# femto-dev/femto

Measured on AMD Instinct MI355X. Metric: patterns/sec (count+locate) on 1 GiB index, higher is better.
Workload: dtype int64

## Files before the change

### femto_amd/build.py

```python
import os
import subprocess
from concurrent.futures import ThreadPoolExecutor

HERE = os.path.dirname(os.path.abspath(__file__))
CSRC = os.path.join(HERE, "csrc")
EXTRACT = os.path.join(HERE, "extract")
DOCLIST = os.path.join(HERE, "doclist")
DOCPOS = os.path.join(HERE, "docpos")
BQUERY = os.path.join(HERE, "bquery")
PLAN = os.path.join(HERE, "plan")
LINES = os.path.join(HERE, "lines")
SIMILAR = os.path.join(HERE, "similar")
MISMATCH = os.path.join(HERE, "mismatch")
EDIT = os.path.join(HERE, "edit")
CLASSES = os.path.join(HERE, "classes")
HAMMING = os.path.join(HERE, "hamming")
COMMON = os.path.join(HERE, "common")
OBJ = os.path.join(HERE, "_obj")
LIB = os.environ.get("FEMTO_AMD_LIB") or os.path.join(HERE, "libfemto_amd.so")
SOURCES = ["femto_amd_api.hip", "api_host.hip", "api_open.hip", "api_multi.hip", "regexp_search.hip", "resolve.hip", "trace_kernels.hip", "host_index.cpp", "index_builder.cpp", "suffix_sort.hip",
           "query_sort.hip", "host_pack.cpp", "../extract/extract.hip", "../doclist/doclist.hip", "../docpos/docpos.hip", "../bquery/bquery.hip", "../plan/plan_stream.hip", "../lines/lines.hip", "../similar/similar.hip", "../mismatch/mismatch.hip", "../edit/edit.hip", "../classes/classes.hip", "../hamming/hamming.hip"]
PLAIN_CXX = {"host_pack.cpp"}
CXX_FLAGS = ["-O3", "-std=c++17", "-fPIC", "-pthread"]
FLAGS = ["--offload-arch=gfx950", "-O3", "-std=c++17", "-fPIC", "-pthread", "-Wno-unused-result", "-Wno-cuda-compat"]
FLAGS += os.environ.get("FEMTO_AMD_EXTRA_FLAGS", "").split()
if os.environ.get("FEMTO_AMD_OBJ"):
    OBJ = os.environ["FEMTO_AMD_OBJ"]


def _headers():
    hs = [os.path.join(d, f) for d in (CSRC, EXTRACT, DOCLIST, DOCPOS, BQUERY, PLAN, LINES, SIMILAR, MISMATCH, EDIT, CLASSES, HAMMING, COMMON) for f in os.listdir(d) if f.endswith((".hpp", ".h"))]
    hs.append(os.path.join(os.path.dirname(HERE), "include", "femto_amd.h"))
    return hs


def _newest_header():
    return max(os.path.getmtime(h) for h in _headers())


def _obj(src):
    return os.path.join(OBJ, os.path.splitext(os.path.basename(src))[0] + ".o")


def _stale(src, hdr_time):
    o = _obj(src)
    if not os.path.exists(o):
        return True
    t = os.path.getmtime(o)
    return os.path.getmtime(os.path.join(CSRC, src)) > t or hdr_time > t


def needs_build():
    if not os.path.exists(LIB):
        return True
    t = os.path.getmtime(LIB)
    if _newest_header() > t:
        return True
    return any(os.path.getmtime(os.path.join(CSRC, f)) > t for f in SOURCES)


def build(force=False, verbose=False):
    if not force and not needs_build():
        return LIB
    os.makedirs(OBJ, exist_ok=True)
    hdr_time = _newest_header()
    todo = [s for s in SOURCES if force or _stale(s, hdr_time)]

    def compile_one(src):
        if src in PLAIN_CXX:
            cmd = ["hipcc"] + CXX_FLAGS + ["-x", "c++", "-c", os.path.join(CSRC, src), "-o", _obj(src)]
        else:
            cmd = ["hipcc"] + FLAGS + ["-x", "hip", "-c", os.path.join(CSRC, src), "-o", _obj(src)]
        if verbose:
            print(" ".join(cmd), flush=True)
        subprocess.run(cmd, check=True)

    with ThreadPoolExecutor(max_workers=min(8, max(1, len(todo)))) as ex:
        list(ex.map(compile_one, todo))
    cmd = ["hipcc", "--offload-arch=gfx950", "-fPIC", "-shared", "-pthread", "-o", LIB] + [_obj(s) for s in SOURCES]
    if verbose:
        print(" ".join(cmd), flush=True)
    subprocess.run(cmd, check=True)
    return LIB


TOOL_SRC = os.path.join(os.path.dirname(HERE), "tools", "femto_amd_multiquery.cpp")
TOOL = os.path.join(HERE, "femto_amd_multiquery")


SEARCH_SRC = os.path.join(os.path.dirname(HERE), "tools", "femto_amd_search.cpp")
SEARCH = os.path.join(HERE, "femto_amd_search")


def build_tools(force=False, verbose=False):
    for src, exe in ((TOOL_SRC, TOOL), (SEARCH_SRC, SEARCH)):
        if not force and os.path.exists(exe) and os.path.getmtime(exe) > max(os.path.getmtime(src), os.path.getmtime(LIB)):
            continue
        cmd = ["g++", "-std=c++17", "-O2", "-o", exe, src, "-L" + HERE, "-lfemto_amd", "-Wl,-rpath,$ORIGIN",
               "-Wl,-rpath-link," + HERE, "-Wl,--allow-shlib-undefined"]
        if verbose:
            print(" ".join(cmd))
        subprocess.run(cmd, check=True)
    return TOOL


if __name__ == "__main__":
    build(force=True, verbose=True)
    build_tools(force=True, verbose=True)
```

### femto_amd/plan/plan_stream.hip

```cpp
#include <algorithm>
#include <atomic>
#include <cstdlib>

#include "../csrc/api_internal.hpp"
#include "../csrc/kernels.hip.hpp"
#include "../csrc/pack_kernels.hip.hpp"
#include "../csrc/ru_kernels.hip.hpp"
#include "../csrc/pack2_kernels.hip.hpp"
#include "../csrc/ind_kernels.hip.hpp"
#include "../csrc/text_kernels.hip.hpp"
#include "../csrc/ctx_kernels.hip.hpp"
#include "../csrc/direct_kernels.hip.hpp"
#include "plan_span.hpp"

namespace femto_amd {
namespace {

struct alignas(16) I64x2 { int64_t x, y; };

__device__ __forceinline__ void wave_lds_sync() {
  __builtin_amdgcn_fence(__ATOMIC_RELEASE, "wavefront");
  __builtin_amdgcn_wave_barrier();
  __builtin_amdgcn_fence(__ATOMIC_ACQUIRE, "wavefront");
}

__device__ __forceinline__ int4 load_counts(const int32_t* __restrict__ noccs, int64_t npats, int64_t t, int64_t t1, int lane) {
  int4 v = make_int4(0, 0, 0, 0);
  if (t >= t1) return v;
  const int64_t q0 = t * kPlanTile + 4 * lane;
  if (q0 + 4 <= npats) {
    v = *reinterpret_cast<const int4*>(noccs + q0);
  } else {
    if (q0 < npats) v.x = noccs[q0];
    if (q0 + 1 < npats) v.y = noccs[q0 + 1];
    if (q0 + 2 < npats) v.z = noccs[q0 + 2];
  }
  return v;
}

__device__ __forceinline__ void load_quad(const int64_t* __restrict__ a, bool vec, int64_t q0, const bool need[4], int64_t out[4]) {
  if (vec) {
    const I64x2 lo = *reinterpret_cast<const I64x2*>(a + q0), hi = *reinterpret_cast<const I64x2*>(a + q0 + 2);
    out[0] = lo.x; out[1] = lo.y; out[2] = hi.x; out[3] = hi.y;
  } else {
#pragma unroll
    for (int j = 0; j < 4; j++) out[j] = need[j] ? a[q0 + j] : 0;
  }
}

template <bool kLong>
__global__ __launch_bounds__(256) __attribute__((amdgpu_waves_per_eu(kLong ? 6 : 8, 8))) void plan_stream_kernel(
    const int64_t npats, const int32_t* __restrict__ noccs, const int64_t* __restrict__ first, const PlanSums ps,
    int64_t* __restrict__ out_starts, int64_t* __restrict__ offsets, const int64_t capacity, int* __restrict__ big_flag,
    const DevIndex ix, int64_t* __restrict__ total_out, int64_t* __restrict__ total_user, const int64_t* __restrict__ sa_known) {
  __shared__ uint32_t s_incl[kPlanWavesPerGroup][kPlanTile];
  __shared__ int64_t s_first[kPlanWavesPerGroup][kPlanTile];
  __shared__ int64_t s_lrel[kLong ? kPlanWavesPerGroup : 1][kLong ? kPlanTile : 1];
  const int lane = threadIdx.x & 63, wv = threadIdx.x >> 6;
  const int64_t nwaves = int64_t(gridDim.x) * kPlanWavesPerGroup, wave = int64_t(blockIdx.x) * kPlanWavesPerGroup + wv;
  for (int64_t k = wave * 64 + lane; k < ps.next_words; k += nwaves * 64) ps.next_super[k] = 0;
  const PlanSpan span = plan_span_of(ps.nblocks, nwaves, wave);
  if (span.t0 >= span.t1) return;
  int4 cur = load_counts(noccs, npats, span.t0, span.t1, lane);
  int4 nx1 = load_counts(noccs, npats, span.t0 + 1, span.t1, lane);
  int64_t base;
  {
    const int64_t b = span.t0, g = b >> 6;
    uint64_t acc = lane < int(b & 63) ? uint64_t(ps.sums[(b & ~int64_t(63)) + lane]) : 0;
    if (lane < int(g & 63)) acc += uint64_t(ps.super[(g & ~int64_t(63)) + lane]);
    for (int64_t k = lane; k < (g >> 6); k += 64) acc += uint64_t(ps.super2[k]);
    const uint64_t part = wave_sum_u64(acc);
    const uint32_t lo = uint32_t(__shfl(int(uint32_t(part)), 0, 64)), hi = uint32_t(__shfl(int(uint32_t(part >> 32)), 0, 64));
    base = int64_t((uint64_t(hi) << 32) | lo);
  }
  const bool first_vec = (reinterpret_cast<uintptr_t>(first) & 15u) == 0, known_vec = (reinterpret_cast<uintptr_t>(sa_known) & 15u) == 0;
  for (int64_t t = span.t0; t < span.t1; t++) {
    const int4 nx2 = load_counts(noccs, npats, t + 2, span.t1, lane);
    const int64_t q0 = t * kPlanTile + 4 * lane;
    const int64_t n[4] = {int64_t(cur.x), int64_t(cur.y), int64_t(cur.z), int64_t(cur.w)};
    const int64_t lsum = n[0] + n[1] + n[2] + n[3];
    int64_t incl = lsum;
    if (kLong) {
      uint64_t v = uint64_t(lsum);
#pragma unroll
      for (int d = 1; d < 64; d <<= 1) {
        const uint32_t lo = uint32_t(__shfl_up(int(uint32_t(v)), d, 64)), hi = uint32_t(__shfl_up(int(uint32_t(v >> 32)), d, 64));
        if (lane >= d) v += (uint64_t(hi) << 32) | lo;
      }
      incl = int64_t(v);
    } else {
      uint32_t v = uint32_t(lsum);
#pragma unroll
      for (int d = 1; d < 64; d <<= 1) {
        const uint32_t y = uint32_t(__shfl_up(int(v), d, 64));
        if (lane >= d) v += y;
      }
      incl = int64_t(v);
    }
    int64_t tile_rows;
    if (kLong) {
      const uint32_t lo = uint32_t(__shfl(int(uint32_t(uint64_t(incl))), 63, 64)), hi = uint32_t(__shfl(int(uint32_t(uint64_t(incl) >> 32)), 63, 64));
      tile_rows = int64_t((uint64_t(hi) << 32) | lo);
    } else {
      tile_rows = int64_t(uint32_t(__shfl(int(uint32_t(incl)), 63, 64)));
    }
    const int64_t rel0 = incl - lsum;
    const int64_t s0 = base + rel0, s1 = s0 + n[0], s2 = s1 + n[1], s3 = s2 + n[2];
    if (q0 + 4 <= npats) {
      *reinterpret_cast<I64x2*>(out_starts + q0) = I64x2{s0, s1};
      *reinterpret_cast<I64x2*>(out_starts + q0 + 2) = I64x2{s2, s3};
    } else {
      if (q0 < npats) out_starts[q0] = s0;
      if (q0 + 1 < npats) out_starts[q0 + 1] = s1;
      if (q0 + 2 < npats) out_starts[q0 + 2] = s2;
    }
    if (offsets && tile_rows > 0) {
      bool live[4], big[4];
      bool any_big = false;
#pragma unroll
      for (int j = 0; j < 4; j++) {
        big[j] = kLong && n[j] > kExpandSerialMax;
        any_big |= big[j];
        live[j] = q0 + j < npats && !big[j] && n[j] > 0;
      }
      if (kLong && any_big) atomicOr(big_flag, 1);
      uint32_t mine[4], linc[4], lsum2 = 0;
#pragma unroll
      for (int j = 0; j < 4; j++) {
        mine[j] = live[j] ? uint32_t(n[j]) : 0u;
        lsum2 += mine[j];
        linc[j] = lsum2;
      }
      uint32_t before = uint32_t(rel0);
      if (kLong) {
        uint32_t v = lsum2;
#pragma unroll
        for (int d = 1; d < 64; d <<= 1) {
          const uint32_t y = uint32_t(__shfl_up(int(v), d, 64));
          if (lane >= d) v += y;
        }
        before = v - lsum2;
      }
      *reinterpret_cast<uint4*>(&s_incl[wv][4 * lane]) = make_uint4(before + linc[0], before + linc[1], before + linc[2], before + linc[3]);
      const uint32_t total = uint32_t(__shfl(int(before + lsum2), 63, 64));
      bool need_known[4], need_first[4], want_known = false, want_first = false;
      int64_t known[4] = {-1, -1, -1, -1}, f[4];
#pragma unroll
      for (int j = 0; j < 4; j++) {
        need_known[j] = sa_known && mine[j] == 1u;
        want_known |= need_known[j];
      }
      const bool whole = q0 + 4 <= npats;
      if (want_known) load_quad(sa_known, whole && known_vec, q0, need_known, known);
#pragma unroll
      for (int j = 0; j < 4; j++) {
        need_first[j] = mine[j] && !(need_known[j] && known[j] >= 0);
        want_first |= need_first[j];
      }
      if (want_first) load_quad(first, whole && first_vec, q0, need_first, f);
#pragma unroll
      for (int j = 0; j < 4; j++) {
        if (!need_first[j]) f[j] = (need_known[j] && known[j] >= 0) ? ~known[j] : 0;
      }
      *reinterpret_cast<I64x2*>(&s_first[wv][4 * lane]) = I64x2{f[0], f[1]};
      *reinterpret_cast<I64x2*>(&s_first[wv][4 * lane + 2]) = I64x2{f[2], f[3]};
      if (kLong) {
        *reinterpret_cast<I64x2*>(&s_lrel[wv][4 * lane]) = I64x2{rel0, rel0 + n[0]};
        *reinterpret_cast<I64x2*>(&s_lrel[wv][4 * lane + 2]) = I64x2{rel0 + n[0] + n[1], rel0 + n[0] + n[1] + n[2]};
      }
      wave_lds_sync();
      for (uint32_t r0 = 0; r0 < total; r0 += 64) {
        const uint32_t sidx = r0 + uint32_t(lane);
        if (sidx < total) {
          int lo = 0, hi = kPlanTile - 1;
          while (lo < hi) {
            const int mid = (lo + hi) >> 1;
            if (s_incl[wv][mid] > sidx) hi = mid; else lo = mid + 1;
          }
          const uint32_t bef = lo ? s_incl[wv][lo - 1] : 0u;
          const int64_t k = int64_t(sidx - bef);
          const int64_t slot = base + (kLong ? s_lrel[wv][lo] : int64_t(bef)) + k;
          if (slot < capacity) {
            const int64_t fr = s_first[wv][lo], row = fr + k;
            if (fr < 0) {
              offsets[slot] = ~fr;
            } else {
              offsets[slot] = sa_at(ix, row);
              trace_touch(ix, kTraceSa, sa_line_of(ix, row));
            }
          }
        }
      }
      wave_lds_sync();
    }
    base += tile_rows;
    cur = nx1;
    nx1 = nx2;
  }
  if (span.t1 == ps.nblocks && lane == 0) {
    total_out[0] = base;
    total_out[1] = base > capacity ? 1 : 0;
    if (total_user) {
      total_user[0] = base;
      total_user[1] = base > capacity ? 1 : 0;
    }
    out_starts[npats] = base;
  }
}

std::atomic<int64_t> g_streamed{0}, g_fell_back{0}, g_big_launches{0}, g_last_groups{0};

int launch_plan_stream(femto_amd_index* ix, Scratch& S, int64_t npats, const int32_t* d_noccs, const int64_t* d_first, int64_t* d_out_starts,
                       int64_t* d_offsets, int64_t capacity, hipStream_t stream, const int64_t* d_sa_known, int max_occs, int64_t forced_groups) {
  int* big_flag = S.d_flags + 1;
  const int64_t ntiles = plan_tiles(npats);
  const PlanSums ps = plan_sums_at(S.bsums.p, ntiles, false, S.bsums_parity);
  S.bsums_clean = true;
  const dim3 grid{uint32_t(plan_stream_groups(ntiles, ix->num_cus, forced_groups))}, block{uint32_t(kBlockThreads)};
  const bool may_be_long = int64_t(max_occs) > kExpandSerialMax;
  hipEvent_t e0 = nullptr, e1 = nullptr;
  timer_begin(ix, ix->t_locate, stream, &e0, &e1);
  if (may_be_long) {
    hipLaunchKernelGGL(plan_stream_kernel<true>, grid, block, 0, stream, npats, d_noccs, d_first, ps, d_out_starts, d_offsets, capacity,
                       big_flag, ix->dev, S.d_total, S.total_user, d_sa_known);
    const dim3 bgrid{uint32_t(std::min<int64_t>(ntiles, int64_t(ix->num_cus) * 8))};
    hipLaunchKernelGGL((plan_big_rows_kernel<kRowsSa, PackPolicy>), bgrid, block, 0, stream, npats, d_first, static_cast<const int2*>(nullptr),
                       static_cast<const int64_t*>(d_out_starts), static_cast<const int64_t*>(S.d_total), capacity, d_offsets,
                       static_cast<const int*>(big_flag), ix->dev);
    g_big_launches++;
  } else {
    hipLaunchKernelGGL(plan_stream_kernel<false>, grid, block, 0, stream, npats, d_noccs, d_first, ps, d_out_starts, d_offsets, capacity,
                       big_flag, ix->dev, S.d_total, S.total_user, d_sa_known);
  }
  HIP_TRY(hipGetLastError());
  timer_end(ix, ix->t_locate, stream, e0, e1);
  g_streamed++;
  g_last_groups = int64_t(grid.x);
  return 0;
}

}
}

int femto_amd_locate_device_v2(femto_amd_index_t* ix, int64_t npats, const int32_t* d_plen, const uint16_t* d_pats,
                               const int64_t* d_starts, int max_occs_each, int64_t* d_first, int64_t* d_last,
                               int32_t* d_noccs, int64_t* d_out_starts, int64_t* d_offsets, int64_t offsets_capacity,
                               int64_t* d_total, void* stream_) {
  API_BEGIN
  bool direct = false;
  const int rc = locate_chain(
      ix, npats, d_plen, d_pats, d_starts, max_occs_each, d_first, d_last, d_noccs, d_out_starts, d_offsets, offsets_capacity, d_total, stream_,
      [&](Scratch& S, const int64_t* first, const Plan& plan, hipStream_t stream) {
        const bool aligned = ((reinterpret_cast<uintptr_t>(d_noccs) | reinterpret_cast<uintptr_t>(d_out_starts)) & 15u) == 0;
        const bool streamed = d_offsets && ix->dev.sa_full && aligned && npats > 0 && knob(-1, "FEMTO_AMD_PLAN_STREAM", 1) != 0;
        if (streamed)
          return launch_plan_stream(ix, S, npats, d_noccs, first, d_out_starts, d_offsets, offsets_capacity, stream, plan.sa_known, max_occs_each,
                                    knob(-1, "FEMTO_AMD_PLAN_STREAM_GRID", 0));
        const int r = launch_plan_rows(ix, S, npats, d_noccs, first, d_out_starts, d_offsets, offsets_capacity, stream, nullptr, true, plan.sa_known);
        if (!r) g_fell_back++;
        return r;
      },
      &direct);
  if (!rc && !direct) g_fell_back++;
  return rc;
  API_END
}

void femto_amd_plan_stream_stats(int64_t out[4]) {
  out[0] = g_streamed.load();
  out[1] = g_fell_back.load();
  out[2] = g_big_launches.load();
  out[3] = g_last_groups.load();
}
```

### include/femto_amd.h

```cpp
#ifndef FEMTO_AMD_H
#define FEMTO_AMD_H

#include <stdint.h>
#include <stddef.h>

#ifdef __cplusplus
extern "C" {
#endif

enum {
  FEMTO_AMD_OK = 0,
  FEMTO_AMD_ERR_MEM = 1,
  FEMTO_AMD_ERR_IO = 2,
  FEMTO_AMD_ERR_PARAM = 3,
  FEMTO_AMD_ERR_FORMAT = 4,
  FEMTO_AMD_ERR_BZ_DATA = 5,
  FEMTO_AMD_ERR_INVALID = 6,
  FEMTO_AMD_ERR_MISSING = 8,
  FEMTO_AMD_ERR_FULL = 10,
  FEMTO_AMD_ERR_OVERWORKED = 11,
  FEMTO_AMD_ERR_UNKNOWN = 12
};

#define FEMTO_AMD_ALPHA_SIZE 261
#define FEMTO_AMD_CHARACTER_OFFSET 5

typedef struct femto_amd_index femto_amd_index_t;

int femto_amd_open(const char* index_path, int device, femto_amd_index_t** out);
void femto_amd_close(femto_amd_index_t* ix);

const char* femto_amd_last_error(void);

typedef struct {
  int64_t total_length;
  int64_t number_of_blocks;
  int64_t number_of_documents;
  int32_t block_size, bucket_size, mark_period, chunk_size;
  int32_t text_size_bits;
  int64_t total_buckets;
  int64_t image_bytes;
  int64_t table_bytes;
} femto_amd_info_t;
int femto_amd_info(const femto_amd_index_t* ix, femto_amd_info_t* out);


int femto_amd_parallel_count(femto_amd_index_t* ix, int npats, const int* plen,
                             const uint16_t* const* pats, int64_t* first, int64_t* last);

int femto_amd_parallel_locate(femto_amd_index_t* ix, int npats, const int* plen,
                              const uint16_t* const* pats, int max_occs_each,
                              int* noccs, int64_t** offsets);

int femto_amd_parallel_locate_range(femto_amd_index_t* ix, int64_t first, int64_t last, int64_t* offsets);

int femto_amd_count_flat(femto_amd_index_t* ix, int64_t npats, const int32_t* plen,
                         const uint16_t* pats, const int64_t* starts, int64_t* first, int64_t* last);
int femto_amd_locate_flat(femto_amd_index_t* ix, int64_t npats, const int32_t* plen,
                          const uint16_t* pats, const int64_t* starts, int max_occs_each,
                          int32_t* noccs, int64_t* out_starts, int64_t* offsets,
                          int64_t offsets_capacity, int64_t* total_out);

int femto_amd_locate_flat_alloc(femto_amd_index_t* ix, int64_t npats, const int32_t* plen,
                                const uint16_t* pats, const int64_t* starts, int max_occs_each,
                                int32_t* noccs, int64_t* out_starts, int64_t** offsets_out, int64_t* total_out);

int femto_amd_count_bytes(femto_amd_index_t* ix, int64_t npats, const int32_t* plen,
                          const uint8_t* bytes, const int64_t* starts, int64_t* first, int64_t* last);

int femto_amd_resolve_location(const femto_amd_index_t* ix, int64_t offset, int64_t* doc, int64_t* doc_offset);
int femto_amd_document_info(const femto_amd_index_t* ix, int64_t doc, const char** info, int64_t* len);

int femto_amd_resolve_batch(femto_amd_index_t* ix, int64_t n, const int64_t* offsets, int64_t* doc, int64_t* doc_offset);

int femto_amd_count_device(femto_amd_index_t* ix, int64_t npats, const int32_t* d_plen,
                           const uint16_t* d_pats, const int64_t* d_starts,
                           int64_t* d_first, int64_t* d_last, void* stream);

int femto_amd_locate_plan_device(femto_amd_index_t* ix, int64_t npats, const int32_t* d_plen,
                                 const uint16_t* d_pats, const int64_t* d_starts, int max_occs_each,
                                 int64_t* d_first, int64_t* d_last, int32_t* d_noccs,
                                 int64_t* d_out_starts, void* stream);
int femto_amd_locate_walk_device(femto_amd_index_t* ix, int64_t npats, const int64_t* d_first,
                                 const int64_t* d_out_starts, int64_t total, int64_t* d_offsets,
                                 void* stream);

int femto_amd_locate_device(femto_amd_index_t* ix, int64_t npats, const int32_t* d_plen,
                            const uint16_t* d_pats, const int64_t* d_starts, int max_occs_each,
                            int64_t* d_first, int64_t* d_last, int32_t* d_noccs, int64_t* d_out_starts,
                            int64_t* d_offsets, int64_t offsets_capacity, int64_t* d_total, void* stream);
int femto_amd_locate_device_v2(femto_amd_index_t* ix, int64_t npats, const int32_t* d_plen,
                               const uint16_t* d_pats, const int64_t* d_starts, int max_occs_each,
                               int64_t* d_first, int64_t* d_last, int32_t* d_noccs, int64_t* d_out_starts,
                               int64_t* d_offsets, int64_t offsets_capacity, int64_t* d_total, void* stream);
void femto_amd_plan_stream_stats(int64_t out[4]);

int femto_amd_lf_steps_device(femto_amd_index_t* ix, int64_t n, const int64_t* d_rows, int64_t* d_next, int64_t* d_off, void* stream);

int femto_amd_resolve_device(femto_amd_index_t* ix, const int64_t* d_offsets, int64_t n, const int64_t* d_n, int64_t* d_doc,
                             int32_t* d_doc32, int64_t* d_doc_offset, void* stream);

typedef struct femto_amd_extractor femto_amd_extractor_t;
#define FEMTO_AMD_EXTRACT_FORCE_SAMPLES 1
#define FEMTO_AMD_EXTRACT_PATH_TEXT 0
#define FEMTO_AMD_EXTRACT_PATH_SAMPLES 1
int femto_amd_extractor_open(femto_amd_index_t* ix, int sample_shift , int flags, femto_amd_extractor_t** out);
void femto_amd_extractor_free(femto_amd_extractor_t* ex);
int femto_amd_extractor_info(const femto_amd_extractor_t* ex, int* path, int* sample_shift, int64_t* bytes, double* build_ms);
int femto_amd_extractor_eof_rows(const femto_amd_extractor_t* ex, int64_t* rows, int64_t n);
int femto_amd_extract_device(femto_amd_extractor_t* ex, int64_t n, const int64_t* d_pos, const int32_t* d_len,
                             const int64_t* d_out_starts, uint16_t* d_out, void* stream);
int femto_amd_context_device(femto_amd_extractor_t* ex, int64_t n, const int64_t* d_rows, const int64_t* d_offsets,
                             const int64_t* d_n, int before, int after, uint16_t* d_ctx, int64_t* d_pos_out, void* stream);
int femto_amd_extract(femto_amd_extractor_t* ex, int64_t n, const int64_t* pos, const int32_t* len, const int64_t* out_starts,
                      uint16_t* out);
int femto_amd_context(femto_amd_extractor_t* ex, int64_t n, const int64_t* rows, const int64_t* offsets, int before, int after,
                      uint16_t* ctx, int64_t* pos_out);
int femto_amd_extract_document(femto_amd_extractor_t* ex, int64_t doc, uint16_t** content, int64_t* len);

#define FEMTO_AMD_LINE_BINARY 1
#define FEMTO_AMD_LINE_INVALID 2
int femto_amd_lines_device(femto_amd_extractor_t* ex, int64_t n, const int64_t* d_offsets, const int64_t* d_n, int64_t* d_doc,
                           int64_t* d_line_pos, int32_t* d_line_len, uint8_t* d_flags, void* stream);
int femto_amd_line_bytes_device(femto_amd_extractor_t* ex, int64_t n, const int64_t* d_n, const int64_t* d_line_pos,
                                const int32_t* d_line_len, int64_t* d_byte_starts , uint8_t* d_bytes, int64_t capacity,
                                int64_t* d_total , void* stream);
int femto_amd_line_groups_device(femto_amd_extractor_t* ex, int64_t n, const int64_t* d_n, const int64_t* d_byte_starts,
                                 const uint8_t* d_bytes, const uint8_t* d_flags, int hash_bits, int64_t* d_group_first,
                                 int64_t* d_ngroups, void* stream);
int femto_amd_lines(femto_amd_extractor_t* ex, int64_t n, const int64_t* offsets, int64_t* doc, int64_t* line_pos, int32_t* line_len,
                    uint8_t* flags, int64_t* byte_starts , uint8_t** bytes, int64_t* total);
int femto_amd_line_groups(femto_amd_extractor_t* ex, int64_t n, const int64_t* byte_starts, const uint8_t* bytes, const uint8_t* flags,
                          int hash_bits, int64_t* group_first, int64_t* ngroups);

#define FEMTO_AMD_DOCSET_AND 0
#define FEMTO_AMD_DOCSET_OR 1
#define FEMTO_AMD_DOCSET_NOT 2
int femto_amd_doclist_info(int* wave_max, int* workgroup_max);
int femto_amd_doclist_device(femto_amd_index_t* ix, int64_t npats, const int64_t* d_out_starts, const int64_t* d_offsets,
                             int64_t capacity, const int64_t* d_total, int32_t* d_ndocs, int64_t* d_docs, int32_t* d_docs32,
                             int32_t* d_hits, int64_t* d_pair_doc, int64_t* d_pair_off, int64_t* d_doc_total, int32_t* d_status,
                             void* stream);
int femto_amd_docset_device(femto_amd_index_t* ix, int64_t npairs, const int64_t* d_docs_a, const int64_t* d_a_start,
                            const int32_t* d_a_n, const int64_t* d_docs_b, const int64_t* d_b_start, const int32_t* d_b_n,
                            const int32_t* d_op, int64_t* d_res_starts , int64_t* d_res_docs, int64_t res_capacity,
                            int64_t* d_res_total , void* stream);
int femto_amd_doclist(femto_amd_index_t* ix, int64_t npats, const int32_t* plen, const uint16_t* pats, const int64_t* starts,
                      int max_occs_each, int64_t* doc_starts , int64_t** docs, int32_t** hits, int64_t* total);
int femto_amd_docset(femto_amd_index_t* ix, int64_t npairs, const int64_t* docs_a, const int64_t* a_start, const int32_t* a_n,
                     const int64_t* docs_b, const int64_t* b_start, const int32_t* b_n, const int32_t* op,
                     int64_t* res_starts , int64_t** res_docs, int64_t* total);

#define FEMTO_AMD_DOCPOS_THEN 0
#define FEMTO_AMD_DOCPOS_WITHIN 1
#define FEMTO_AMD_DOCPOS_OR 2
int femto_amd_docpos_info(int* tile);
int femto_amd_docpos_chunks(void);
int femto_amd_docpos_device(femto_amd_index_t* ix, int64_t npairs, const int64_t* d_a_doc, const int64_t* d_a_off,
                            const int64_t* d_a_start, const int32_t* d_a_n, const int64_t* d_b_doc, const int64_t* d_b_off,
                            const int64_t* d_b_start, const int32_t* d_b_n, const int32_t* d_op, const int32_t* d_distance,
                            int64_t* d_res_starts , int64_t* d_res_doc, int64_t* d_res_off, int64_t res_capacity,
                            int64_t* d_res_total , void* stream);
int femto_amd_docpos_documents_device(femto_amd_index_t* ix, int64_t nlists, const int64_t* d_starts ,
                                      const int64_t* d_pair_doc, int64_t* d_doc_starts , int64_t* d_docs,
                                      int64_t doc_capacity, int64_t* d_total , void* stream);
int femto_amd_docpos(femto_amd_index_t* ix, int64_t npairs, const int64_t* a_doc, const int64_t* a_off, const int64_t* a_start,
                     const int32_t* a_n, const int64_t* b_doc, const int64_t* b_off, const int64_t* b_start, const int32_t* b_n,
                     const int32_t* op, const int32_t* distance, int64_t* res_starts , int64_t** res_doc,
                     int64_t** res_off, int64_t* total);
int femto_amd_proximity(femto_amd_index_t* ix, int64_t npairs, const int32_t* l_plen, const uint16_t* l_pats, const int64_t* l_starts,
                        const int32_t* r_plen, const uint16_t* r_pats, const int64_t* r_starts, const int32_t* op,
                        const int32_t* distance, int max_occs_each, int64_t* res_starts , int64_t** res_doc,
                        int64_t** res_off, int64_t* total);

int femto_amd_match_stats_device(femto_amd_index_t* ix, int64_t n, const uint8_t* d_bytes, int32_t max_len, int32_t* d_len,
                                 int64_t* d_first, int64_t* d_last, void* stream);
int femto_amd_match_stats_steps_device(femto_amd_index_t* ix, int64_t n, const uint8_t* d_bytes, int32_t max_len,
                                       int64_t* d_steps , void* stream);
int femto_amd_common_sequences_device(femto_amd_index_t* ix, int64_t n, const int32_t* d_len, const int64_t* d_first,
                                      const int64_t* d_last, int32_t min_len, int64_t* d_seq_start, int32_t* d_seq_len,
                                      int64_t* d_seq_first, int64_t* d_seq_last, int64_t capacity, int64_t* d_total ,
                                      void* stream);
int femto_amd_common_groups_device(femto_amd_index_t* ix, int64_t capacity, const int64_t* d_total, const int64_t* d_seq_start,
                                   const int32_t* d_seq_len, const int64_t* d_seq_first, const int64_t* d_seq_last,
                                   int64_t* d_group_of, int32_t* d_g_len, int64_t* d_g_first, int64_t* d_g_last, int32_t* d_g_here,
                                   int64_t* d_g_min_start, int64_t* d_ngroups ,
                                   void* stream);
int femto_amd_similar_documents_device(femto_amd_index_t* ix, int64_t ngroups_capacity, const int64_t* d_ngroups,
                                       const int32_t* d_g_len, const int64_t* d_g_first, const int64_t* d_g_last,
                                       const int32_t* d_g_here, const uint8_t* d_g_keep, int max_occs_each, int64_t* d_offsets,
                                       int64_t offsets_capacity, int64_t* d_doc_score, int32_t* d_doc_seqs, int64_t* d_total ,
                                       void* stream);
typedef struct femto_amd_similar_result {
  int64_t n;
  int32_t* len;
  int64_t ngroups;
  int32_t* g_len;
  int64_t* g_first;
  int64_t* g_last;
  int32_t* g_here;
  int64_t* g_min_start;
  uint8_t* g_kept;
  int64_t index_numerator;
  double index_score;
  int64_t ndocs;
  int64_t* doc;
  int64_t* doc_numerator;
  int32_t* doc_seqs;
  double* doc_score;
} femto_amd_similar_result_t;
int femto_amd_similar(femto_amd_index_t* ix, const uint8_t* bytes, int64_t n, int32_t min_len, int32_t max_len, int max_occs_each,
                      int n_not, femto_amd_index_t* const* not_ix, femto_amd_similar_result_t* out);
void femto_amd_similar_free(femto_amd_similar_result_t* out);

int femto_amd_mismatch_device(femto_amd_index_t* ix, int64_t npat, int64_t nsyms, const uint16_t* d_syms,
                              const int64_t* d_starts , int k, int64_t capacity, int64_t* d_result_start ,
                              int64_t* d_first, int64_t* d_last, int32_t* d_cost, int32_t* d_sub_pos ,
                              uint16_t* d_sub_sym , int64_t* d_total , void* stream);
typedef struct femto_amd_mismatch_result {
  int64_t npat;
  int64_t total;
  int64_t* result_start;
  int64_t* first;
  int64_t* last;
  int32_t* cost;
  int32_t* sub_pos;
  uint16_t* sub_sym;
} femto_amd_mismatch_result_t;
int femto_amd_mismatch(femto_amd_index_t* ix, int64_t npat, const int32_t* plen, const uint16_t* syms, int k,
                       femto_amd_mismatch_result_t* out);
void femto_amd_mismatch_free(femto_amd_mismatch_result_t* out);

int femto_amd_edit_device(femto_amd_index_t* ix, int64_t npat, int64_t nsyms, const uint16_t* d_syms,
                          const int64_t* d_starts , int k, int64_t capacity, int64_t* d_result_start ,
                          int64_t* d_first, int64_t* d_last, int32_t* d_cost, int32_t* d_length, int64_t* d_total , void* stream);
typedef struct femto_amd_edit_result {
  int64_t npat;
  int64_t total;
  int64_t* result_start;
  int64_t* first;
  int64_t* last;
  int32_t* cost;
  int32_t* length;
} femto_amd_edit_result_t;
int femto_amd_edit(femto_amd_index_t* ix, int64_t npat, const int32_t* plen, const uint16_t* syms, int k,
                   femto_amd_edit_result_t* out);
void femto_amd_edit_free(femto_amd_edit_result_t* out);

// ... 196 lines not shown
```

Measured before the change: 20.20 billion.

## Add one-round tail count kernel that verifies short SA ranges against text

Adds a dedicated dense count kernel that, once the backward-search range is small, switches to comparing the remaining pattern directly against the text at each candidate suffix. It does this in 16-byte pieces using an LDS-staged translated pattern window, then jumps to the ISA rank, all in a single launch that also emits plan sums and known SA positions. The v2 locate entry point routes eligible dense cases through this path before the existing plan/stream stage, bypassing the older locate chain. This is meant to cut the remaining rank/LF steps and extra rounds, at the cost of more LDS per block, unaligned text reads and a more complex kernel.

```diff
diff --git a/femto_amd/build.py b/femto_amd/build.py
--- a/femto_amd/build.py
+++ b/femto_amd/build.py
@@ -15,11 +15,12 @@
 EDIT = os.path.join(HERE, "edit")
 CLASSES = os.path.join(HERE, "classes")
 HAMMING = os.path.join(HERE, "hamming")
+TAIL = os.path.join(HERE, "tail")
 COMMON = os.path.join(HERE, "common")
 OBJ = os.path.join(HERE, "_obj")
 LIB = os.environ.get("FEMTO_AMD_LIB") or os.path.join(HERE, "libfemto_amd.so")
 SOURCES = ["femto_amd_api.hip", "api_host.hip", "api_open.hip", "api_multi.hip", "regexp_search.hip", "resolve.hip", "trace_kernels.hip", "host_index.cpp", "index_builder.cpp", "suffix_sort.hip",
-           "query_sort.hip", "host_pack.cpp", "../extract/extract.hip", "../doclist/doclist.hip", "../docpos/docpos.hip", "../bquery/bquery.hip", "../plan/plan_stream.hip", "../lines/lines.hip", "../similar/similar.hip", "../mismatch/mismatch.hip", "../edit/edit.hip", "../classes/classes.hip", "../hamming/hamming.hip"]
+           "query_sort.hip", "host_pack.cpp", "../extract/extract.hip", "../doclist/doclist.hip", "../docpos/docpos.hip", "../bquery/bquery.hip", "../plan/plan_stream.hip", "../lines/lines.hip", "../similar/similar.hip", "../mismatch/mismatch.hip", "../edit/edit.hip", "../classes/classes.hip", "../hamming/hamming.hip", "../tail/tail_round.hip"]
 PLAIN_CXX = {"host_pack.cpp"}
 CXX_FLAGS = ["-O3", "-std=c++17", "-fPIC", "-pthread"]
 FLAGS = ["--offload-arch=gfx950", "-O3", "-std=c++17", "-fPIC", "-pthread", "-Wno-unused-result", "-Wno-cuda-compat"]
@@ -29,7 +30,7 @@
 
 
 def _headers():
-    hs = [os.path.join(d, f) for d in (CSRC, EXTRACT, DOCLIST, DOCPOS, BQUERY, PLAN, LINES, SIMILAR, MISMATCH, EDIT, CLASSES, HAMMING, COMMON) for f in os.listdir(d) if f.endswith((".hpp", ".h"))]
+    hs = [os.path.join(d, f) for d in (CSRC, EXTRACT, DOCLIST, DOCPOS, BQUERY, PLAN, LINES, SIMILAR, MISMATCH, EDIT, CLASSES, HAMMING, TAIL, COMMON) for f in os.listdir(d) if f.endswith((".hpp", ".h"))]
     hs.append(os.path.join(os.path.dirname(HERE), "include", "femto_amd.h"))
     return hs
 
diff --git a/femto_amd/plan/plan_stream.hip b/femto_amd/plan/plan_stream.hip
--- a/femto_amd/plan/plan_stream.hip
+++ b/femto_amd/plan/plan_stream.hip
@@ -12,6 +12,7 @@
 #include "../csrc/ctx_kernels.hip.hpp"
 #include "../csrc/direct_kernels.hip.hpp"
 #include "plan_span.hpp"
+#include "../tail/tail_round.hpp"
 
 namespace femto_amd {
 namespace {
@@ -247,20 +248,38 @@
                                int32_t* d_noccs, int64_t* d_out_starts, int64_t* d_offsets, int64_t offsets_capacity,
                                int64_t* d_total, void* stream_) {
   API_BEGIN
+  const auto plan_done = [&](Scratch& S, const int64_t* first, const Plan& plan, hipStream_t stream) {
+    const bool aligned = ((reinterpret_cast<uintptr_t>(d_noccs) | reinterpret_cast<uintptr_t>(d_out_starts)) & 15u) == 0;
+    const bool streamed = d_offsets && ix->dev.sa_full && aligned && npats > 0 && knob(-1, "FEMTO_AMD_PLAN_STREAM", 1) != 0;
+    if (streamed)
+      return launch_plan_stream(ix, S, npats, d_noccs, first, d_out_starts, d_offsets, offsets_capacity, stream, plan.sa_known, max_occs_each,
+                                knob(-1, "FEMTO_AMD_PLAN_STREAM_GRID", 0));
+    const int r = launch_plan_rows(ix, S, npats, d_noccs, first, d_out_starts, d_offsets, offsets_capacity, stream, nullptr, true, plan.sa_known);
+    if (!r) g_fell_back++;
+    return r;
+  };
+  const bool row_free = !d_first && !d_last;
+  const bool valid = ix && !(reinterpret_cast<uintptr_t>(d_pats) & 1u) && max_occs_each >= 0 && offsets_capacity >= 0 && npats > 0 &&
+                     (row_free || (d_first && d_last)) && d_noccs && d_out_starts && d_total;
+  if (valid && !ensure_device(ix) && tail_round_applies(ix, npats, row_free)) {
+    hipStream_t stream = static_cast<hipStream_t>(stream_);
+    Lease L(ix, stream);
+    if (!L.s) return L.rc;
+    Scratch& S = *L.s;
+    Plan plan{max_occs_each, d_noccs, d_out_starts, offsets_capacity, false, d_total};
+    plan.row_free = row_free;
+    int rc;
+    if (row_free) {
+      if ((rc = S.first.reserve(size_t(npats + 1) * 8))) return rc;
+      d_first = S.first.as<int64_t>();
+    }
+    if ((rc = launch_count_tail_round(ix, S, npats, d_plen, d_pats, d_starts, d_first, d_last, stream, &plan))) return rc;
+    return plan_done(S, d_first, plan, stream);
+  }
+  tail_round_fell_back();
   bool direct = false;
-  const int rc = locate_chain(
-      ix, npats, d_plen, d_pats, d_starts, max_occs_each, d_first, d_last, d_noccs, d_out_starts, d_offsets, offsets_capacity, d_total, stream_,
-      [&](Scratch& S, const int64_t* first, const Plan& plan, hipStream_t stream) {
-        const bool aligned = ((reinterpret_cast<uintptr_t>(d_noccs) | reinterpret_cast<uintptr_t>(d_out_starts)) & 15u) == 0;
-        const bool streamed = d_offsets && ix->dev.sa_full && aligned && npats > 0 && knob(-1, "FEMTO_AMD_PLAN_STREAM", 1) != 0;
-        if (streamed)
-          return launch_plan_stream(ix, S, npats, d_noccs, first, d_out_starts, d_offsets, offsets_capacity, stream, plan.sa_known, max_occs_each,
-                                    knob(-1, "FEMTO_AMD_PLAN_STREAM_GRID", 0));
-        const int r = launch_plan_rows(ix, S, npats, d_noccs, first, d_out_starts, d_offsets, offsets_capacity, stream, nullptr, true, plan.sa_known);
-        if (!r) g_fell_back++;
-        return r;
-      },
-      &direct);
+  const int rc = locate_chain(ix, npats, d_plen, d_pats, d_starts, max_occs_each, d_first, d_last, d_noccs, d_out_starts, d_offsets, offsets_capacity,
+                              d_total, stream_, plan_done, &direct);
   if (!rc && !direct) g_fell_back++;
   return rc;
   API_END
diff --git a/femto_amd/tail/tail_piece.hpp b/femto_amd/tail/tail_piece.hpp
--- /dev/null
+++ b/femto_amd/tail/tail_piece.hpp
@@ -0,0 +1,85 @@
+#pragma once
+#include <cstdint>
+
+#if defined(__HIPCC__) || defined(__CUDACC__)
+#define TAIL_PIECE_FN __host__ __device__ inline
+#else
+#define TAIL_PIECE_FN inline
+#endif
+
+namespace femto_amd {
+
+constexpr int kTailPiece = 16;
+constexpr int kTailMaxPieces = 4;
+
+struct TailWords { uint64_t a, b; };
+
+TAIL_PIECE_FN int tail_pieces(int n) { return (n + kTailPiece - 1) / kTailPiece; }
+
+TAIL_PIECE_FN int tail_chunk(int left, int pieces_max) { return left < pieces_max * kTailPiece ? left : pieces_max * kTailPiece; }
+
+TAIL_PIECE_FN int64_t tail_piece_at(int64_t p, int i) { return p - int64_t(kTailPiece) * (i + 1); }
+
+TAIL_PIECE_FN int tail_piece_width(int n) { return n <= 4 ? 4 : (n <= 8 ? 8 : kTailPiece); }
+
+TAIL_PIECE_FN int64_t tail_chunk_low(int64_t p, int n) {
+  return n <= 8 ? p - tail_piece_width(n) : tail_piece_at(p, tail_pieces(n) - 1);
+}
+
+TAIL_PIECE_FN bool tail_round_ok(int64_t p, int n) { return n > 0 && tail_chunk_low(p, n) >= 0; }
+
+TAIL_PIECE_FN uint64_t tail_bswap64(uint64_t v) { return __builtin_bswap64(v); }
+
+TAIL_PIECE_FN TailWords tail_text_words(uint64_t lo, uint64_t hi) { return TailWords{tail_bswap64(hi), tail_bswap64(lo)}; }
+
+TAIL_PIECE_FN uint32_t tail_align(uint32_t hi, uint32_t lo, uint32_t sh) { return uint32_t(((uint64_t(hi) << 32) | lo) >> (8u * (sh & 3u))); }
+
+TAIL_PIECE_FN TailWords tail_window_words(const uint32_t w[5], uint32_t sh) {
+  return TailWords{uint64_t(tail_align(w[1], w[0], sh)) | (uint64_t(tail_align(w[2], w[1], sh)) << 32),
+                   uint64_t(tail_align(w[3], w[2], sh)) | (uint64_t(tail_align(w[4], w[3], sh)) << 32)};
+}
+
+TAIL_PIECE_FN uint64_t tail_mask(int n) { return n >= 8 ? ~uint64_t(0) : (n <= 0 ? uint64_t(0) : (uint64_t(1) << (8 * n)) - 1); }
+
+TAIL_PIECE_FN int tail_piece_diff(const TailWords& win, const TailWords& txt, int n) {
+  const uint64_t xa = (win.a ^ txt.a) & tail_mask(n), xb = (win.b ^ txt.b) & tail_mask(n - 8);
+  if (xa) return (__builtin_ffsll(static_cast<long long>(xa)) - 1) >> 3;
+  if (xb) return 8 + ((__builtin_ffsll(static_cast<long long>(xb)) - 1) >> 3);
+  return n;
+}
+
+struct TailPieceBytes { uint64_t lo, hi; };
+
+template <int kPieces, class Win, class Txt>
+TAIL_PIECE_FN int tail_chunk_match(int n, uint32_t k, Win&& win, Txt&& txt) {
+  static_assert(kPieces >= 1 && kPieces <= kTailMaxPieces, "a chunk is one to four pieces");
+  const int np = tail_pieces(n);
+  TailPieceBytes t[kPieces];
+#pragma unroll
+  for (int i = 0; i < kPieces; i++)
+    if (i < np) t[i] = txt(i);
+  const uint32_t d = k >> 2, sh = k & 3u;
+#pragma unroll
+  for (int i = 0; i < kPieces; i++) {
+    if (i < np) {
+      const uint32_t d0 = d + 4u * uint32_t(i);
+      const uint32_t w[5] = {win(d0), win(d0 + 1u), win(d0 + 2u), win(d0 + 3u), sh ? win(d0 + 4u) : 0u};
+      const int ni = n - kTailPiece * i < kTailPiece ? n - kTailPiece * i : kTailPiece;
+      const int df = tail_piece_diff(tail_window_words(w, sh), tail_text_words(t[i].lo, t[i].hi), ni);
+      if (df < ni) return kTailPiece * i + df;
+    }
+  }
+  return n;
+}
+
+template <class Win, class Txt>
+TAIL_PIECE_FN int tail_short_match(int n, uint32_t k, Win&& win, Txt&& txt) {
+  const uint64_t t = txt(tail_piece_width(n));
+  const uint32_t d = k >> 2, sh = k & 3u;
+  const uint32_t w0 = win(d), w1 = win(d + 1u), w2 = sh ? win(d + 2u) : 0u;
+  const uint64_t a = uint64_t(tail_align(w1, w0, sh)) | (uint64_t(tail_align(w2, w1, sh)) << 32);
+  const uint64_t x = (a ^ tail_bswap64(t)) & tail_mask(n);
+  return x ? (__builtin_ffsll(static_cast<long long>(x)) - 1) >> 3 : n;
+}
+
+}
diff --git a/femto_amd/tail/tail_round.hip b/femto_amd/tail/tail_round.hip
--- /dev/null
+++ b/femto_amd/tail/tail_round.hip
@@ -0,0 +1,332 @@
+#include <atomic>
+
+#include "../csrc/api_internal.hpp"
+#include "../csrc/kernels.hip.hpp"
+#include "../csrc/pack_kernels.hip.hpp"
+#include "../csrc/ru_kernels.hip.hpp"
+#include "../csrc/pack2_kernels.hip.hpp"
+#include "../csrc/ind_kernels.hip.hpp"
+#include "../csrc/text_kernels.hip.hpp"
+#include "../csrc/ctx_kernels.hip.hpp"
+#include "../csrc/direct_kernels.hip.hpp"
+#include "../csrc/direct_launch.hpp"
+#include "tail_piece.hpp"
+#include "tail_round.hpp"
+
+namespace femto_amd {
+
+template <class P, bool kPlan, bool kDense, int kPieces>
+__global__ __launch_bounds__(256) __attribute__((amdgpu_waves_per_eu(P::kDirectWaves, P::kDirectWaves))) void count_direct_kernel(
+    const DevIndex ix, const int64_t npats, const int32_t* __restrict__ plen, const uint16_t* __restrict__ pats,
+    const int64_t* __restrict__ starts, int64_t* __restrict__ first_out, int64_t* __restrict__ last_out, int* __restrict__ err_flag,
+    const int max_occs, int32_t* __restrict__ noccs, const PlanSums ps, int* __restrict__ big_flag, int64_t* __restrict__ sa_out) {
+  static_assert(kPlan && kDense, "the one-round tail exists for dense launches with a plan");
+  constexpr int kWinDw = 18, kWin = 4 * kWinDw;
+  static_assert(kTailPiece * kPieces + 7 < kWin, "a chunk after a refill fits the window");
+  constexpr bool kShortLoads = !std::is_same<P, PackPolicy>::value;
+  __shared__ uint16_t s_code[264];
+  __shared__ uint8_t s_byte[264];
+  __shared__ int64_t s_w[4];
+  __shared__ uint32_t s_win[kWinDw * 256];
+  const int64_t q = int64_t(blockIdx.x) * blockDim.x + threadIdx.x;
+  const int len_q = q < npats ? plen[q] : 0;
+  const int64_t start_q = q < npats ? starts[q] : 0;
+  for (int i = threadIdx.x; i < 264; i += blockDim.x) {
+    const uint32_t c = i < kAlphaSize ? uint32_t(P::code_of(ix, uint32_t(i))) : 0xffffu;
+    s_code[i] = uint16_t(c);
+    s_byte[i] = uint8_t((c < 255u && !P::is_stop(ix, c)) ? c : 0xFFu);
+  }
+  __syncthreads();
+  int64_t nocc = 0;
+  if (q < npats) {
+    const int len = len_q;
+    const uint16_t* pat = pats + start_q;
+    auto phase = [&]() -> int { return int(((reinterpret_cast<uintptr_t>(pat) >> 1) + uintptr_t(uint32_t(len))) & 7u); };
+    int w0 = -(1 << 30);
+    uint8_t* const win = reinterpret_cast<uint8_t*>(s_win);
+    auto waddr = [&](uint32_t k) -> uint32_t { return (((k >> 2) * 256u + threadIdx.x) << 2) + (k & 3u); };
+    auto tr4 = [&](const uint32_t a, const uint32_t b) -> uint32_t {
+      auto T = [&](uint32_t sym) -> uint32_t { return s_byte[sym < 263u ? sym : 263u]; };
+      return T(b >> 16) | (T(b & 0xffffu) << 8) | (T(a >> 16) << 16) | (T(a & 0xffffu) << 24);
+    };
+    auto fill_at = [&](const int nw0, auto batch) {
+      constexpr int kB = decltype(batch)::value;
+      w0 = nw0;
+      int emax = (len - 1 - nw0) >> 3;
+      emax = emax < kWinDw / 2 - 1 ? emax : kWinDw / 2 - 1;
+      const uint16_t* const gp0 = pat + (len - 8 - nw0);
+#pragma unroll 1
+      for (int e0 = 0; e0 <= emax; e0 += kB) {
+        uint4 v[kB];
+#pragma unroll
+        for (int i = 0; i < kB; i++)
+          if (e0 + i <= emax) v[i] = *reinterpret_cast<const uint4*>(gp0 - 8 * (e0 + i));
+#pragma unroll
+        for (int i = 0; i < kB; i++)
+          if (e0 + i <= emax) {
+            s_win[uint32_t(2 * (e0 + i)) * 256u + threadIdx.x] = tr4(v[i].z, v[i].w);
+            s_win[uint32_t(2 * (e0 + i) + 1) * 256u + threadIdx.x] = tr4(v[i].x, v[i].y);
+          }
+      }
+    };
+    if (len > 0) fill_at(-((8 - phase()) & 7), std::integral_constant<int, 4>{});
+    auto refill = [&](int j) { fill_at(j - ((j - phase()) & 7), std::integral_constant<int, 2>{}); };
+    auto wcode = [&](int j) -> uint32_t {
+      if (j < w0 || j >= w0 + kWin) refill(j);
+      return win[waddr(uint32_t(j - w0))];
+    };
+    auto alpha = [&](int j) -> uint32_t { return pat[len - 1 - j]; };
+    int64_t first = 0, last = ix.total_length - 1;
+    int64_t sa_hint = -1;
+    int j = 0;
+    if (ix.ctx && len >= ix.ctx_syms) {
+      const int H1 = ix.ctx_syms, H2 = (ix.ctx2 && len >= ix.ctx2_syms) ? ix.ctx2_syms : 0;
+      const int HM = (ix.ctxm && len >= ix.ctxm_syms) ? ix.ctxm_syms : 0;
+      const int HH = H2 ? H2 : (HM ? HM : H1);
+      const uint32_t nstop = uint32_t(ix.ctx_nstop);
+      const int bits = ix.ctx_bits;
+      uint64_t key1 = 0;
+      CtxKey2 key2{0, 0};
+      int okn = 0;
+      for (; okn < HH; okn++) {
+        const uint32_t code = wcode(okn);
+        if (code == 0xFFu) break;
+        const uint64_t field = uint64_t(code - nstop + 1u);
+        if (okn < H1) key1 |= field << (bits * okn);
+        if (H2 | HM) ctx_key2_or(key2, field, bits * okn);
+      }
+      if (H2 && okn == H2 && ctx2_lookup(ix, key2, first, last, &sa_hint) == 1) j = H2;
+      else if (HM && okn >= HM && ctxm_lookup(ix, key2, first, last, &sa_hint) == 1) j = HM;
+      else if (okn >= H1 && ctx_lookup(ix, key1, first, last) == 1) j = H1;
+      if (j == 0 || j == H1) sa_hint = -1;
+    }
+    if (j == 0 && ix.ktab2) {
+      const int kmax = len < ix.kt2_syms ? len : ix.kt2_syms;
+      const uint32_t nstop = uint32_t(ix.kt2_nstop);
+      const int64_t t = ix.kt2_base;
+      int64_t pos = 0;
+      for (; j < kmax; j++) {
+        const uint32_t code = wcode(j);
+        if (code == 0xFFu) break;
+        pos = pos * t + 1 + int64_t(code - nstop);
+      }
+      ktab2_lookup<P>(ix, pos, j, first, last, &sa_hint);
+      if (first > last) j = len;
+    }
+    bool tried = false, finished = false;
+    int ones = 0;
+    const bool row_free = ix.row_free != 0;
+    int rf = 0;
+    int need_ones = ix.tail_ones;
+    if (need_ones > 0) {
+      const unsigned long long act = __ballot(1), alive = __ballot(first <= last && j < len);
+      if (__popcll(alive) * 4 >= __popcll(act) * 3) need_ones = 0;
+    }
+    const bool fast_cmp = P::max_code(ix) < 255u;
+    for (;;) {
+      for (; j < len; j++) {
+        if (!tried && last - first < int64_t(P::kTailRows) && last - first < int64_t(ix.tail_rows) && j > 0 && ones >= need_ones &&
+            len - j >= ix.tail_min + ix.tail_row_cost * int(last - first)) break;
+        if (row_free && !tried && sa_hint >= 0 && first == last) break;
+        uint32_t code = wcode(j);
+        if (code == 0xFFu) {
+          const uint32_t ch = alpha(j);
+          if (ch >= uint32_t(kAlphaSize)) {
+            atomicOr(err_flag, 1);
+            first = 0;
+            last = -1;
+            finished = true;
+            break;
+          }
+          code = s_code[ch];
+          if (code == 0xffffu) {
+            first = ix.C[ch];
+            last = first - 1;
+            finished = true;
+            break;
+          }
+        }
+        P::search_step(ix, j, code, first, last);
+        sa_hint = -1;
+        if (first > last) { finished = true; break; }
+        tried = false;
+        ones = first == last ? ones + 1 : 0;
+      }
+      if (finished || j >= len) break;
+      tried = true;
+      const int remaining = len - j;
+      int best = 0;
+      int64_t qmin = 0, qmax = -1;
+      int64_t pbest = -1;
+      for (int64_t row = first; row <= last; row++) {
+        int64_t p = sa_hint;
+        if (!(row == first && sa_hint >= 0)) {
+          p = sa_at(ix, row);
+          trace_touch(ix, kTraceSa, sa_line_of(ix, row));
+        }
+        if (p <= 0 || p >= ix.total_length) continue;
+        const int lim = p < int64_t(remaining) ? int(p) : remaining;
+        const uint8_t* const tp = ix.txt + (p - 1);
+        int m = 0;
+        bool stopped = false;
+        if (fast_cmp) {
+          while (m < lim) {
+            const int n = tail_chunk(lim - m, kPieces);
+            const int64_t low = kShortLoads ? tail_chunk_low(p - m, n) : tail_piece_at(p - m, tail_pieces(n) - 1);
+            if (low < 0) break;
+            const int jj = j + m;
+            if (jj < w0 || jj + kTailPiece * tail_pieces(n) > w0 + kWin) refill(jj);
+            const uint8_t* const t0 = ix.txt + (p - m);
+            trace_touch_span(ix, kTraceTxt, uint64_t(low), uint64_t(p - m - 1));
+            const auto window = [&](uint32_t d) -> uint32_t { return s_win[d * 256u + threadIdx.x]; };
+            int eq;
+            if (kShortLoads && n <= 8) {
+              eq = tail_short_match(n, uint32_t(jj - w0), window, [&](int w) -> uint64_t {
+                uint64_t v;
+                if (w == 8) {
+                  __builtin_memcpy(&v, t0 - 8, 8);
+                } else {
+                  uint32_t u;
+                  __builtin_memcpy(&u, t0 - 4, 4);
+                  v = uint64_t(u) << 32;
+                }
+                return v;
+              });
+            } else {
+              eq = tail_chunk_match<kPieces>(n, uint32_t(jj - w0), window, [&](int i) -> TailPieceBytes {
+                TailPieceBytes b;
+                __builtin_memcpy(&b, t0 - kTailPiece * (i + 1), sizeof b);
+                return b;
+              });
+            }
+            m += eq;
+            if (eq < n) {
+              stopped = true;
+              break;
+            }
+          }
+        }
+        if (!stopped)
+          for (; m < lim; m++) {
+            const uint32_t code = wcode(j + m);
+            if (code == 0xFFu) break;
+            trace_touch(ix, kTraceTxt, uint64_t(tp - m - ix.txt) >> 7);
+            if (uint32_t(tp[-m]) != code) break;
+          }
+        if (row_free && first == last) {
+          if (m == remaining) {
+            rf = 1;
+            pbest = p - m;
+            break;
+          }
+          if (m < lim) {
+            const uint32_t code = wcode(j + m);
+            if (code != 0xFFu && uint32_t(tp[-m]) != code) {
+              rf = 2;
+              break;
+            }
+          }
+        }
+        if (m > 0 && m >= best && ix.isa_shift == 0) {
+          const int64_t q2 = isa_at(ix, p - m);
+          trace_touch(ix, kTraceIsa, sa_line_of(ix, p - m));
+          if (m > best) {
+            best = m;
+            qmin = qmax = q2;
+            pbest = p - m;
+          } else {
+            qmin = q2 < qmin ? q2 : qmin;
+            qmax = q2 > qmax ? q2 : qmax;
+          }
+        }
+      }
+      sa_hint = -1;
+      if (rf == 1) {
+        sa_hint = pbest;
+        break;
+      }
+      if (rf == 2) {
+        first = 0;
+        last = -1;
+        break;
+      }
+      if (best > 0) {
+        first = qmin;
+        last = qmax;
+        j += best;
+        if (qmin == qmax) sa_hint = pbest;
+      }
+      if (j >= len) break;
+    }
+    if (ix.row_free) {
+    } else if (last_out) {
+      first_out[q] = first;
+      last_out[q] = last;
+    } else {
+      first_out[q] = last - first + 1;
+    }
+    if (first > last) nocc = 0;
+    else if (last - first > int64_t(max_occs)) nocc = max_occs;
+    else nocc = last - first + 1;
+    noccs[q] = int32_t(nocc);
+    if (ix.row_free && nocc > 0 && rf != 1) first_out[q] = first;
+    if (sa_out) {
+      if (__ballot(nocc == 1)) sa_out[q] = first == last ? sa_hint : -1;
+    }
+  }
+  const int64_t s = block_sum_256(nocc, s_w);
+  if (threadIdx.x == 0) {
+    ps.sums[blockIdx.x] = s;
+    if (ps.acc && s) {
+      atomicAdd(reinterpret_cast<unsigned long long*>(&ps.super[blockIdx.x >> 6]), static_cast<unsigned long long>(s));
+      atomicAdd(reinterpret_cast<unsigned long long*>(&ps.super2[blockIdx.x >> 12]), static_cast<unsigned long long>(s));
+    }
+    if (blockIdx.x == 0 && big_flag) *big_flag = 0;
+  }
+}
+
+namespace {
+std::atomic<int64_t> g_round{0}, g_old_chain{0};
+}
+
+bool tail_round_applies(const femto_amd_index* ix, int64_t npats, bool row_free) {
+  return use_direct(ix) && npats > 0 && npats <= (int64_t(1) << 31) && direct_decision(ix->mode, ix->dev, true, row_free).dense &&
+         knob(-1, "FEMTO_AMD_TAIL_ROUND", 1) != 0;
+}
+
+void tail_round_fell_back() { g_old_chain++; }
+
+int launch_count_tail_round(femto_amd_index* ix, Scratch& S, int64_t npats, const int32_t* d_plen, const uint16_t* d_pats, const int64_t* d_starts,
+                            int64_t* d_first, int64_t* d_last, hipStream_t stream, Plan* plan) {
+  const int64_t nblocks = direct_blocks(npats);
+  DevIndex d = ix->dev;
+  int rc;
+  inline_tail_setup(ix, d);
+  d.row_free = plan->row_free ? 1 : 0;
+  if ((rc = reserve_plan_sums(S, nblocks, true, stream))) return rc;
+  const PlanSums ps = plan_sums_at(S.bsums.p, nblocks, true, S.bsums_parity);
+  if ((rc = S.noccs64.reserve(size_t(npats + 1) * 8))) return rc;
+  int64_t* const sa_out = S.noccs64.as<int64_t>();
+  plan->sa_known = sa_out;
+  hipEvent_t e0 = nullptr, e1 = nullptr;
+  timer_begin(ix, ix->t_count, stream, &e0, &e1);
+  const dim3 grid{uint32_t(nblocks)}, block{256};
+  const bool known = with_policy<RumPolicy, RuPolicy, PackPolicy, IndPolicy, Pack2Policy>(rank_kind(ix->mode, d), [&](auto tag) {
+    using P = typename decltype(tag)::type;
+    hipLaunchKernelGGL((count_direct_kernel<P, true, true, kTailRoundPieces>), grid, block, 0, stream, d, npats, d_plen, d_pats, d_starts, d_first, d_last,
+                       S.err, plan->max_occs, plan->noccs, ps, S.d_flags + 1, sa_out);
+  });
+  HIP_TRY(known ? hipGetLastError() : hipErrorInvalidDeviceFunction);
+  timer_end(ix, ix->t_count, stream, e0, e1);
+  S.total_user = plan->total_user;
+  plan->done = true;
+  g_round++;
+  return 0;
+}
+
+}
+
+void femto_amd_tail_round_stats(int64_t out[2]) {
+  out[0] = femto_amd::g_round.load();
+  out[1] = femto_amd::g_old_chain.load();
+}
diff --git a/femto_amd/tail/tail_round.hpp b/femto_amd/tail/tail_round.hpp
--- /dev/null
+++ b/femto_amd/tail/tail_round.hpp
@@ -0,0 +1,16 @@
+#pragma once
+#include "../csrc/api_internal.hpp"
+
+namespace femto_amd {
+
+constexpr int kTailRoundPieces = 2;
+
+int reserve_plan_sums(Scratch& S, int64_t nblocks, bool fold, hipStream_t stream);
+void inline_tail_setup(const femto_amd_index* ix, DevIndex& d);
+
+bool tail_round_applies(const femto_amd_index* ix, int64_t npats, bool row_free);
+int launch_count_tail_round(femto_amd_index* ix, Scratch& S, int64_t npats, const int32_t* d_plen, const uint16_t* d_pats, const int64_t* d_starts,
+                            int64_t* d_first, int64_t* d_last, hipStream_t stream, Plan* plan);
+void tail_round_fell_back();
+
+}
diff --git a/include/femto_amd.h b/include/femto_amd.h
--- a/include/femto_amd.h
+++ b/include/femto_amd.h
@@ -94,6 +94,7 @@
                                int64_t* d_first, int64_t* d_last, int32_t* d_noccs, int64_t* d_out_starts,
                                int64_t* d_offsets, int64_t offsets_capacity, int64_t* d_total, void* stream);
 void femto_amd_plan_stream_stats(int64_t out[4]);
+void femto_amd_tail_round_stats(int64_t out[2]);
 
 int femto_amd_lf_steps_device(femto_amd_index_t* ix, int64_t n, const int64_t* d_rows, int64_t* d_next, int64_t* d_off, void* stream);
 
```

Measured after the change: 20.19 billion, median of 4. About the same (-0.0%).
